# barry-mir/mixing-style-transfer

Measured on AMD Instinct MI355X. Metric: triplets/sec (10 s @ 44.1 kHz, 4-stem, bs=24), higher is better.
Workload: dtype f32

## Files before the change

mixing-style-transfer_amd/csrc/encoder.hip:

```cpp
#include "common.h"

#include <cmath>
#include <type_traits>
#include <vector>

namespace {

typedef float f32x4 __attribute__((ext_vector_type(4)));
constexpr int kConvThreads = 512;
constexpr int kConvWaves = 8;

struct FilmParams {
  const float* feats;
  const float *w0t, *b0, *w3t, *b3, *hwt, *hb;
  const float *s1, *t1, *s2, *t2;
  float* film;
  float2* aff1;
  float2* aff2;
  int Fd, H, nsub;
};

#ifndef MST_FILM_U
#define MST_FILM_U 4
#endif
// ... 90 lines not shown
  static constexpr int RL = 16;
};

template <int SUB>
struct CC<3, SUB> {
  static constexpr int CIN = 64, COUT = 32, NCH = 16, MT = 5, NT = 2;
  static constexpr int WIN = 10, WPG = 2;
  static constexpr int TROWS = 2, TCOLS = 40;
  static constexpr int PR = TROWS + 6, PC = TCOLS + 6;
  static constexpr int RL = 64;
};

template <int SUB>
struct CC<4, SUB> {
  static constexpr int CIN = 32, COUT = 64, NCH = 8, MT = 5, NT = 4;
  static constexpr int WIN = 10, WPG = 2;
  static constexpr int TROWS = 2, TCOLS = 40;
  static constexpr int PR = TROWS + 6, PC = TCOLS + 6;
  static constexpr int RL = 64;
};

struct ConvParams {
  const float* in;
  const float* wfrag;
  const float2* aff;
  float* out;
  int B, nsub;
  int in_rows, in_cols;
  int in_cstride;
  int in_bandoff;
  long long in_clipstride;
  int out_rows, out_cols;
  int tiles_r, tiles_c;
  int sets_per_band;
  float* yraw;
  mst::DetAcc* stats;
  const float* bias;
  int raw_rows, raw_cols;
  const unsigned char* mask;
  float mask_scale;
  int acc_tr, acc_tc, row_off;
  const float* f16_scale;
  const float* f16_winv;
  int pool_h;
  int clip_major;
  _Float16* yraw16;
  const float* y_scale;
  const void* in_lo;
  int cm_mels, cm_overlap;
};

typedef _Float16 h16x4 __attribute__((ext_vector_type(4)));
__device__ __forceinline__ size_t yvec(size_t unit, int t, int nvec) {
  return (unit & ~(size_t)63) * nvec + (size_t)t * 64 + (unit & 63);
}
template <int NV>
__device__ __forceinline__ void load_unit(const void* yraw, const float* y_scale, int band, size_t unit, float (&v)[NV]) {
  if (y_scale) {
    const float inv = y_scale[band * 2 + 1];
    const h16x4* s = reinterpret_cast<const h16x4*>(yraw);
#pragma unroll
    for (int t = 0; t < NV / 4; ++t) {
      const h16x4 q = s[yvec(unit, t, NV / 4)];
#pragma unroll
      for (int r = 0; r < 4; ++r) v[4 * t + r] = (float)q[r] * inv;
    }
// ... 58 lines not shown
  constexpr int WBP = GEO::WBP, PATCH = GEO::PATCH, NWF = GEO::NWF, NPF = GEO::NPF, NCV = GEO::NCV;
  constexpr bool BL = LAYER == 2;
  constexpr int NPFK = BL ? 16 : NPF;
  constexpr int NPIECE = NPFK + NWF, PPT = (NPIECE + 48) / 49;
  extern __shared__ __attribute__((aligned(16))) float smem[];
  const int tid = threadIdx.x, lane = tid & 63;
  const int wave = __builtin_amdgcn_readfirstlane(tid >> 6);
  float* wbuf = smem;
  float* pbuf = smem + 2 * WBP + wave * PATCH;

  const int G = gridDim.x;
  const int wg = mst::xcd_remap(blockIdx.x, G);
  const int total_sets = p.nsub * p.sets_per_band;
  constexpr bool CONTIG = MODE == 1 || MODE == 3;
  const int s_first = CONTIG ? (int)((long long)wg * total_sets / G) : wg;
  const int my_sets = CONTIG ? (int)((long long)(wg + 1) * total_sets / G) - s_first
                             : (wg < total_sets ? (total_sets - wg + G - 1) / G : 0);
  const int nq = my_sets * NCH;
  const int tpb = p.tiles_r * p.tiles_c;

  auto decode = [&](int q) __attribute__((always_inline)) {
    const int s = CONTIG ? min(s_first + q / NCH, total_sets - 1) : wg + (q / NCH) * G;
    Tile t;
    t.band = min(s / p.sets_per_band, p.nsub - 1);
    const int idx = (s - t.band * p.sets_per_band) * kConvWaves + wave;
    t.valid = (q < nq) && idx < p.B * tpb;
    t.clip = t.valid ? idx / tpb : 0;
    const int ti = t.valid ? idx - t.clip * tpb : 0;
    t.tc = ti / p.tiles_r;
    t.tr = ti - t.tc * p.tiles_r;
    return t;
  };

  constexpr bool TS = LAYER == 2 && MODE == 0;
  const int kq = lane >> 4, ai = lane & 15, ag = ai >> 2, areg = ai & 3;
  int abase[MT];
#pragma unroll
  for (int t = 0; t < MT; ++t) {
    int dr, wc;
    if constexpr (GEO1) {
      const int e = 4 * t + areg, wv = e / C::WIN, pos = e % C::WIN;
      dr = pos / 5;
      wc = 5 * (C::WPG * ag + wv) + pos % 5;
    } else {
      dr = TS ? 2 * t + (ag >> 1) : 4 * (ag >> 1) + t;
      wc = 4 * (ag & 1) + areg;
    }
    abase[t] = kq * (PR * PC) + dr * PC + wc;
  }

  f32x4 wreg[NWF];
  float pf[NPFK];
  unsigned long long rowmask = 0;
  unsigned colmask = 0;
  int coff[NCV];
  const float* nsrc = p.in;
  const f32x4* nwsrc = reinterpret_cast<const f32x4*>(p.wfrag);
  int nrow0 = 0, ncol0 = 0, nvalid = 0;
  __amdgpu_buffer_rsrc_t nrsrc = __builtin_amdgcn_make_buffer_rsrc(const_cast<float*>(p.in), 0, 0, 0x00020000);
  __amdgpu_buffer_rsrc_t nwrsrc = __builtin_amdgcn_make_buffer_rsrc(const_cast<float*>(p.wfrag), 0, 0, 0x00020000);
  unsigned nvoff[4] = {0, 0, 0, 0}, nsoff[4] = {0, 0, 0, 0};

  auto prefetch_setup = [&](int q, const Tile& t) __attribute__((always_inline)) {
    const int chunk = q % NCH;
    nwsrc = reinterpret_cast<const f32x4*>(p.wfrag + ((size_t)t.band * NCH + chunk) * WBP);
    nrow0 = (GEO1 ? C::TROWS * t.tr : 8 * t.tr) + (MODE == 3 ? p.row_off : 0) - 3;
    ncol0 = C::TCOLS * t.tc - 3;
    nvalid = t.valid;
    nsrc = p.in + (size_t)t.clip * p.in_clipstride + (size_t)t.band * p.in_bandoff + (size_t)(4 * chunk) * p.in_cstride;
    rowmask = 0, colmask = 0;
    if constexpr (BL) {
      nrsrc = __builtin_amdgcn_make_buffer_rsrc(const_cast<float*>(nsrc), 0, (unsigned)(4 * p.in_cstride) * 4u, 0x00020000);
      nwrsrc = __builtin_amdgcn_make_buffer_rsrc(const_cast<f32x4*>(nwsrc), 0, (unsigned)WBP * 4u, 0x00020000);
      if (chunk == 0) {
        const int rs = lane >> 4, col = lane & 15, cin = ncol0 + col;
        const bool col_in = nvalid && col < PC && cin >= 0 && cin < p.in_cols;
        const int cbase = max(ncol0, 0);
#pragma unroll
// ... 27 lines not shown
        const int row = i / NCV, j = i % NCV;
        const int cc = row / PR, r = row % PR;
        const int rin = nrow0 + r;
        const int rc = min(max(rin, 0), p.in_rows - 1);
        if (nvalid && rin == rc) rowmask |= 1ull << i;
        const float* rowp = nsrc + (size_t)cc * p.in_cstride + (size_t)rc * p.in_cols;
        pf[i] = rowp[coff[j]];
      } else {
        const int e = lane + 64 * i;
        const int row = e / RL, col = e % RL;
        const int cc = min(row / PR, 3), r = row % PR;
        const int rin = nrow0 + r, cin = ncol0 + col;
        const int rc = min(max(rin, 0), p.in_rows - 1), cl = min(max(cin, 0), p.in_cols - 1);
        if (nvalid && row < 4 * PR && col < PC && rin == rc && cin == cl) colmask |= 1u << i;
        pf[i] = nsrc[cc * p.in_cstride + rc * p.in_cols + cl];
      }
    } else if (i < NPIECE) {
      wreg[i - NPF] = nwsrc[tid + kConvThreads * (i - NPF)];
    }
  };

  f32x4 acc[MT][NT];
  double st[NT][2];
  int st_band = -1;
#pragma unroll
  for (int n = 0; n < NT; ++n) st[n][0] = st[n][1] = 0.0;
  Tile cur{}, nxt{};
  nxt = decode(0);
  if (nq > 0) {
    prefetch_setup(0, nxt);
#pragma unroll
    for (int i = 0; i < NPIECE; ++i) prefetch_piece(i);
  }
#ifdef MST_TRACE
  long long trc[5] = {0, 0, 0, 0, 0};
  const long long trc_start = clock64();
#endif
  for (int q = 0; q < nq; ++q) {
    float* wb = wbuf + (q & 1) * WBP;
#ifdef MST_TRACE
    const long long tq0 = clock64();
#endif
#pragma unroll
    for (int i = 0; i < NWF; ++i) reinterpret_cast<f32x4*>(wb)[tid + kConvThreads * i] = wreg[i];
    if constexpr (BL) {
#pragma unroll
      for (int i = 0; i < NPFK; ++i) {
        const int rs = lane >> 4, col = lane & 15, r = 4 * (i & 3) + rs;
        if (r < PR && col < PC) pbuf[((i >> 2) * PR + r) * PC + col] = pf[i];
      }
    } else
#pragma unroll
    for (int i = 0; i < NPF; ++i) {
      if constexpr (RL >= 64) {
        const int row = i / NCV, j = i % NCV, col = lane + 64 * j;
        const bool ok = ((rowmask >> i) & 1ull) && ((colmask >> j) & 1u);
        if (col < PC) pbuf[row * PC + col] = ok ? pf[i] : 0.f;
      } else {
        const int e = lane + 64 * i;
        const int row = e / RL, col = e % RL;
        if (row < 4 * PR && col < PC) pbuf[row * PC + col] = ((colmask >> i) & 1u) ? pf[i] : 0.f;
      }
    }
#ifdef MST_TRACE
    asm volatile("s_waitcnt lgkmcnt(0)" ::: "memory");
    const long long tq1 = clock64();
#endif
    __syncthreads();
#ifdef MST_TRACE
    const long long tq2 = clock64();
    trc[0] += tq1 - tq0, trc[1] += tq2 - tq1, trc[4] += 1;
#endif
    cur = nxt;
    if (!BL || (q + 1) % NCH == 0) nxt = decode(q + 1);
    prefetch_setup(q + 1, nxt);
    const int chunk = q % NCH;
    if (chunk == 0) {
#pragma unroll
      for (int t = 0; t < MT; ++t)
#pragma unroll
        for (int n = 0; n < NT; ++n) acc[t][n] = f32x4{0.f, 0.f, 0.f, 0.f};
    }
    {
      float a[2][MT], b[2][NT];
#pragma unroll
      for (int t = 0; t < MT; ++t) a[0][t] = pbuf[abase[t]];
#pragma unroll
      for (int n = 0; n < NT; ++n) b[0][n] = wb[n * 64 + lane];
      auto taps = [&](auto LO_, auto HI_, auto SKIP_) __attribute__((always_inline)) {
        constexpr int LO = decltype(LO_)::value, HI = decltype(HI_)::value;
        constexpr bool SKIP0 = decltype(SKIP_)::value;
#pragma unroll
        for (int tap = LO; tap < HI; ++tap) {
          const int cu = tap & 1, nx = cu ^ 1;
          const int off = ((tap + 1) / 7) * PC + ((tap + 1) % 7);
#pragma unroll
          for (int i = 0; i < MT * NT; ++i) {
            const int t = i / NT, n = i % NT;
            if (!(SKIP0 && t == 0)) acc[t][n] = __builtin_amdgcn_mfma_f32_16x16x4f32(a[cu][t], b[cu][n], acc[t][n], 0, 0, 0);
            if (tap + 1 < 49) {
              if (i < NT) b[nx][i] = wb[((tap + 1) * NT + i) * 64 + lane];
              else if (i < MT + NT) a[nx][i - NT] = pbuf[abase[i - NT] + off];
            }
            if (i >= MT + NT && i - (MT + NT) < PPT) prefetch_piece(tap * PPT + (i - (MT + NT)));
            __builtin_amdgcn_sched_barrier(0);
          }
        }
      };
      using I0 = std::integral_constant<int, 0>;
      using I14 = std::integral_constant<int, 14>;
      using I49 = std::integral_constant<int, 49>;
      if constexpr (TS) {
        if (cur.tr == 0) taps(I0{}, I14{}, std::true_type{});
        else taps(I0{}, I14{}, std::false_type{});
        taps(I14{}, I49{}, std::false_type{});
      } else {
        taps(I0{}, I49{}, std::false_type{});
      }
    }
#ifdef MST_TRACE
    trc[2] += clock64() - tq2;
#endif
    if (MODE == 1 && chunk == NCH - 1 && cur.valid) {
      const int j = lane & 15, g = lane >> 4;
      if (cur.band != st_band) {
        if (st_band >= 0) flush_stats<NT, C::COUT>(st, p.stats, st_band, lane);
        st_band = cur.band;
      }
      float* yb = p.yraw + ((((size_t)cur.clip * p.nsub + cur.band) * p.acc_tr + cur.tr) * p.acc_tc + cur.tc) *
                               (size_t)(NT * 64 * 4 * MT);
#pragma unroll
      for (int n = 0; n < NT; ++n) {
        const float b = p.bias[cur.band * C::COUT + n * 16 + j];
        f32x4* dst = reinterpret_cast<f32x4*>(yb) + (size_t)n * (64 * MT) + lane;
#pragma unroll
        for (int t = 0; t < MT; ++t) {
          f32x4 v = acc[t][n];
#pragma unroll
          for (int r = 0; r < 4; ++r) {
            v[r] += b;
            int row, col;
            if constexpr (LAYER == 1) {
              const int e = 4 * t + r, wv = e / C::WIN, pos = e % C::WIN;
              row = C::TROWS * cur.tr + pos / 5, col = C::TCOLS * cur.tc + 5 * (C::WPG * g + wv) + pos % 5;
            } else {
              row = 8 * cur.tr + 4 * (g >> 1) + t, col = 8 * cur.tc + 4 * (g & 1) + r;
            }
            if (row < p.raw_rows && col < p.raw_cols) st[n][0] += (double)v[r], st[n][1] += (double)v[r] * (double)v[r];
          }
          dst[64 * t] = v;
        }
      }
    }
    if (MODE == 3 && chunk == NCH - 1 && cur.valid) {
      const int j = lane & 15, g = lane >> 4;
// ... 32 lines not shown
          const int wv = e / C::WIN, pos = e % C::WIN;
          const int row = C::TROWS * cur.tr + pos / 5, col = C::TCOLS * cur.tc + 5 * (C::WPG * g + wv) + pos % 5;
          if (row < p.raw_rows && col < p.raw_cols) {
            const size_t o = (size_t)row * p.raw_cols + col;
            float v = acc[e >> 2][n][e & 3];
            if (mb) v = mb[o] ? v * p.mask_scale : 0.f;
            ob[o] = v;
          }
        }
      }
    }
    if (MODE == 0 && chunk == NCH - 1 && cur.valid) {
      const int j = lane & 15, g = lane >> 4;
      const float2* aff = p.aff + ((size_t)cur.clip * p.nsub + cur.band) * C::COUT;
#pragma unroll
      for (int n = 0; n < NT; ++n) {
        const int ch = n * 16 + j;
        const float2 ac = aff[ch];
        if constexpr (LAYER == 1) {
#pragma unroll
          for (int wv = 0; wv < C::WPG; ++wv) {
            float m = 0.f;
#pragma unroll
            for (int pos = 0; pos < C::WIN; ++pos) {
              const int e = wv * C::WIN + pos;
              m = fmaxf(m, fmaf(acc[e >> 2][n][e & 3], ac.x, ac.y));
            }
            const int pc = 4 * C::WPG * cur.tc + C::WPG * g + wv;
            if (pc < p.out_cols)
              p.out[((((size_t)cur.clip * p.nsub + cur.band) * C::COUT + ch) * p.out_rows + cur.tr) * p.out_cols + pc] = m;
          }
        } else {
          float m = 0.f;
          if constexpr (TS) {
            float m0 = 0.f, m1 = 0.f;
#pragma unroll
            for (int r = 0; r < 4; ++r) {
              m0 = fmaxf(m0, fmaxf(fmaf(acc[0][n][r], ac.x, ac.y), fmaf(acc[1][n][r], ac.x, ac.y)));
              m1 = fmaxf(m1, fmaxf(fmaf(acc[2][n][r], ac.x, ac.y), fmaf(acc[3][n][r], ac.x, ac.y)));
            }
            m0 = fmaxf(m0, __shfl_xor(m0, 32, 64));
            m1 = fmaxf(m1, __shfl_xor(m1, 32, 64));
            m = (g >> 1) ? m1 : m0;
          } else {
#pragma unroll
            for (int t = 0; t < MT; ++t)
#pragma unroll
              for (int r = 0; r < 4; ++r) m = fmaxf(m, fmaf(acc[t][n][r], ac.x, ac.y));
          }
          const int pr = 2 * cur.tr + (g >> 1), pc = 2 * cur.tc + (g & 1);
          if (pr < p.out_rows && pc < p.out_cols)
            p.out[(((size_t)cur.clip * p.nsub + cur.band) * C::COUT + ch) * p.out_rows * p.out_cols +
                  (size_t)pr * p.out_cols + pc] = m;
        }
      }
    }
  }
#ifdef MST_TRACE
  if (MODE == 0 && LAYER == 2 && lane == 0 && p.yraw) {
    float* o = p.yraw + (blockIdx.x * kConvWaves + wave) * 8;
    for (int i = 0; i < 5; ++i) o[i] = (float)trc[i];
    o[5] = (float)(clock64() - trc_start);
  }
#endif
  if ((MODE == 1 || MODE == 3) && st_band >= 0) flush_stats<NT, C::COUT>(st, p.stats, st_band, lane);
}

template <int SUB, int MODE = 0, int LAY = 0>
__global__ __launch_bounds__(kConvThreads) void conv1_resident_kernel(const ConvParams p) {
  using C = CC<1, SUB>;
  constexpr int MT = C::MT, NT = C::NT, PR = C::PR, PC = C::PC;
  static_assert(C::RL == 64, "resident conv1 expects one loader row per instruction");
  static_assert(LAY == 0 || PR == 8, "the channel-minor loader maps lane bits 1..3 to the 8 patch rows");
  constexpr int WCH = 49 * NT * 64;
  constexpr int WBP = ConvGeom<1, SUB>::WBP;
  constexpr int CHS = PR * PC;
  constexpr int PATCH = 8 * CHS;
  constexpr int NPF = LAY == 0 ? 8 * PR : (PC + 3) / 4;
  extern __shared__ __attribute__((aligned(16))) float smem[];
  const int tid = threadIdx.x, lane = tid & 63;
  const int wave = __builtin_amdgcn_readfirstlane(tid >> 6);
  float* wres = smem;
  float* pbuf = smem + 2 * WCH + wave * PATCH;
  constexpr bool DYN = MODE == 0;
  constexpr int kTickets = 16;
  __shared__ unsigned tickets[kTickets];
#ifdef MST_TRACE
  long long trc[5] = {0, 0, 0, 0, 0};
  const long long trc_start = clock64();
#endif

  const int G = gridDim.x;
  const int wg = mst::xcd_remap(blockIdx.x, G);
  const int total_sets = (p.clip_major ? (p.B + p.clip_major - 1) / p.clip_major : 1) * p.nsub * p.sets_per_band;
  const int s_begin = (int)((long long)wg * total_sets / G), s_end = (int)((long long)(wg + 1) * total_sets / G);
  const int tpb = p.tiles_r * p.tiles_c;

  auto decode = [&](int s) __attribute__((always_inline)) {
    Tile t;
    int ti;
    if (p.clip_major) {
      const int ngrp = (p.B + p.clip_major - 1) / p.clip_major;
      const int gb = min(s / p.sets_per_band, ngrp * p.nsub - 1);
      const int idx = (s - gb * p.sets_per_band) * kConvWaves + wave;
      const int grp = gb / p.nsub, c0 = grp * p.clip_major;
      t.band = gb - grp * p.nsub;
      t.valid = (s < s_end) && idx < min(p.clip_major, p.B - c0) * tpb;
      const int cl = t.valid ? idx / tpb : 0;
      t.clip = c0 + cl;
      ti = t.valid ? idx - cl * tpb : 0;
    } else {
      t.band = min(s / p.sets_per_band, p.nsub - 1);
      const int idx = (s - t.band * p.sets_per_band) * kConvWaves + wave;
      t.valid = (s < s_end) && idx < p.B * tpb;
      t.clip = t.valid ? idx / tpb : 0;
      ti = t.valid ? idx - t.clip * tpb : 0;
    }
    t.tc = ti / p.tiles_r;
    t.tr = ti - t.tc * p.tiles_r;
    return t;
  };

  const int kq = lane >> 4, ai = lane & 15, ag = ai >> 2, areg = ai & 3;
  int abase[MT];
#pragma unroll
  for (int t = 0; t < MT; ++t) {
    const int e = 4 * t + areg, wv = e / C::WIN, pos = e % C::WIN;
    abase[t] = kq * CHS + (pos / 5) * PC + 5 * (C::WPG * ag + wv) + pos % 5;
  }

  typename std::conditional<LAY == 0, float, f32x4>::type pf[NPF];
  unsigned long long rowmask = 0;
  bool col_ok = false;
  int coff = 0, nrow0 = 0, nvalid = 0;
  const float* nsrc = p.in;
  bool nfast = false;
  __amdgpu_buffer_rsrc_t nrsrc = __builtin_amdgcn_make_buffer_rsrc(const_cast<float*>(p.in), 0, 0, 0x00020000);
  unsigned nsoff = 0, nvoff = 0;
  static_assert(WBP - WCH >= 4, "the chunk pitch leaves at least 16 zero bytes behind the weights");
  const float* const zero16 = p.wfrag + WCH;
  const int lr = (lane >> 1) & 7, lhalf = lane & 1, lfq = lane >> 4;
  const unsigned frame_bytes = (unsigned)p.cm_mels * 32u;
  auto prefetch_setup = [&](const Tile& t) __attribute__((always_inline)) {
    nrow0 = C::TROWS * t.tr - 3;
    nvalid = t.valid;
    rowmask = 0;
    if constexpr (LAY == 0) {
      const int col0 = C::TCOLS * t.tc - 3, cin = col0 + lane;
      nsrc = p.in + (size_t)t.clip * p.in_clipstride + (size_t)t.band * p.in_bandoff;
      col_ok = lane < PC && cin >= 0 && cin < p.in_cols;
      coff = min(max(cin, 0), p.in_cols - 1);
    } else {
      const int rin = nrow0 + lr, rc = min(max(rin, 0), p.in_rows - 1);
      nsrc = p.in + (size_t)t.clip * p.in_clipstride;
      col_ok = nvalid && rin == rc;
      coff = ((t.band * p.cm_overlap + rc) * 8 + 4 * lhalf) * 4;
      nrow0 = C::TCOLS * t.tc - 3 + lfq;
      if constexpr (DYN) {
        const int f0 = C::TCOLS * t.tc - 3;
        nfast = nvalid && f0 >= 0 && f0 + 4 * NPF + 3 < p.in_cols;
        nrsrc = __builtin_amdgcn_make_buffer_rsrc(const_cast<float*>(nsrc), 0, (unsigned)p.in_cols * frame_bytes, 0x00020000);
// ... 199 lines not shown
            }
          } else {
            float m = 0.f;
#pragma unroll
            for (int pos = 0; pos < C::WIN; ++pos) {
              const int e = wv * C::WIN + pos;
              m = fmaxf(m, fmaf(acc[e >> 2][n][e & 3], ac.x, ac.y));
            }
            if (pc < p.out_cols) orow[(size_t)ch * p.out_rows * p.out_cols + pc] = m;
          }
        }
      }
    }
#ifdef MST_TRACE
    trc[1] += clock64() - tr1;
#endif
  };
  f32x4 sav[MT][NT];
  float2 sav_ac[NT];
  Tile prev{};
#pragma unroll
  for (int t = 0; t < MT; ++t)
#pragma unroll
    for (int n = 0; n < NT; ++n) sav[t][n] = f32x4{0.f, 0.f, 0.f, 0.f};
#pragma unroll
  for (int n = 0; n < NT; ++n) sav_ac[n] = float2{0.f, 0.f};
  auto epi_part = [&](auto N_, auto WV_) __attribute__((always_inline)) {
    constexpr int n = decltype(N_)::value, wv = decltype(WV_)::value;
    const int j = lane & 15, g = lane >> 4;
    const int ch = n * 16 + j;
    float* orow = p.out + ((size_t)prev.clip * p.nsub + prev.band) * C::COUT * p.out_rows * p.out_cols + (size_t)prev.tr * p.out_cols;
    const float2 ac = sav_ac[n];
    const int pc = 4 * C::WPG * prev.tc + C::WPG * g + wv;
    if (SUB == 2 && p.pool_h == 1) {
#pragma unroll
      for (int hr = 0; hr < 2; ++hr) {
        float m = 0.f;
#pragma unroll
        for (int pos = 0; pos < 5; ++pos) {
          const int e = wv * C::WIN + 5 * hr + pos;
          m = fmaxf(m, fmaf(sav[e >> 2][n][e & 3], ac.x, ac.y));
        }
        if (prev.valid && pc < p.out_cols && 2 * prev.tr + hr < p.out_rows)
          orow[(size_t)ch * p.out_rows * p.out_cols + (size_t)(prev.tr + hr) * p.out_cols + pc] = m;
      }
    } else {
      float m = 0.f;
#pragma unroll
      for (int pos = 0; pos < C::WIN; ++pos) {
        const int e = wv * C::WIN + pos;
        m = fmaxf(m, fmaf(sav[e >> 2][n][e & 3], ac.x, ac.y));
      }
      if (prev.valid && pc < p.out_cols) orow[(size_t)ch * p.out_rows * p.out_cols + pc] = m;
    }
  };
  auto tile_dyn = [&]() __attribute__((always_inline)) {
#ifdef MST_TRACE
    const long long tr0 = clock64();
#endif
    float2 e_ac[NT];
    {
      const float2* aff = p.aff + ((size_t)cur.clip * p.nsub + cur.band) * C::COUT;
#pragma unroll
      for (int n = 0; n < NT; ++n) e_ac[n] = aff[n * 16 + (lane & 15)];
    }
    {
      constexpr int kEpi0 = 12;
      const bool skip_c = cur.tr == 0, skip_b = 2 * cur.tr + 2 >= p.in_rows;
      const int next_off = skip_b ? 0 : 5 * PC, next_w = skip_b ? 0 : 35 * NT * 64;
      float a[2][MT], b[2][NT];
#pragma unroll
      for (int t = 0; t < MT; ++t) a[0][t] = pbuf[abase[t] + 2 * PC];
#pragma unroll
      for (int n = 0; n < NT; ++n) b[0][n] = wres[(14 * NT + n) * 64 + lane];
      auto kstep = [&](auto S_) __attribute__((always_inline)) {
        constexpr int ks = decltype(S_)::value;
        constexpr int cu = ks & 1, nx = cu ^ 1;
        constexpr bool last = ks == 41 || ks == 69 || ks == 97;
        constexpr int s1 = ks + 1, l1 = s1 < 42 ? s1 : s1 < 70 ? s1 - 42 : s1 - 70;
        constexpr int row1 = (s1 < 42 ? 2 : s1 < 70 ? 5 : 0) + l1 / 14, tap1 = 7 * row1 + (l1 % 14) / 2, ch1 = l1 & 1;
        constexpr int off1 = ch1 * 4 * CHS + row1 * PC + (l1 % 14) / 2;
#pragma unroll
        for (int i = 0; i < MT * NT; ++i) {
          const int t = i / NT, n = i % NT;
          acc[t][n] = __builtin_amdgcn_mfma_f32_16x16x4f32(a[cu][t], b[cu][n], ks == 0 ? f32x4{0.f, 0.f, 0.f, 0.f} : acc[t][n], 0, 0, 0);
          if constexpr (!last) {
            if (i < NT) b[nx][i] = wres[ch1 * WCH + (tap1 * NT + i) * 64 + lane];
            else if (i < MT + NT) a[nx][i - NT] = pbuf[abase[i - NT] + off1];
          } else if constexpr (ks == 41) {
            if (i < NT) b[nx][i] = wres[next_w + i * 64 + lane];
            else if (i < MT + NT) a[nx][i - NT] = pbuf[abase[i - NT] + next_off];
          } else if constexpr (ks == 69) {
            if (i < NT) b[nx][i] = wres[i * 64 + lane];
            else if (i < MT + NT) a[nx][i - NT] = pbuf[abase[i - NT]];
          }
          if (i == MT + NT) {
            if constexpr (LAY == 0) {
              if constexpr (ks >= 8 && ks < 8 + NPF / 2) prefetch_piece(2 * (ks - 8)), prefetch_piece(2 * (ks - 8) + 1);
            } else {
              if constexpr (ks >= 8 && ks % 2 == 0 && ks / 2 - 4 < NPF) prefetch_piece(ks / 2 - 4);
            }
          }
          if (i == MT + NT + 1) {
            if constexpr (ks == 0) ticket_issue();
            if constexpr (ks == 6) {
              nxt = ticket_take();
              nxt_seg = dseg;
              prefetch_setup(nxt);
            }
            if constexpr (ks >= kEpi0 && ks < kEpi0 + 2 * NT * C::WPG && (ks - kEpi0) % 2 == 0)
              epi_part(std::integral_constant<int, (ks - kEpi0) / 2 / C::WPG>{}, std::integral_constant<int, (ks - kEpi0) / 2 % C::WPG>{});
          }
          __builtin_amdgcn_sched_barrier(0);
        }
      };
      static_assert(LAY == 0 ? 8 + NPF / 2 <= 42 : 2 * (NPF + 3) < 42, "the patch fetch must fit block A");
      static_for<42>([&](auto I) __attribute__((always_inline)) { kstep(std::integral_constant<int, decltype(I)::value>{}); });
      if (!skip_b) static_for<28>([&](auto I) __attribute__((always_inline)) { kstep(std::integral_constant<int, 42 + decltype(I)::value>{}); });
      if (!skip_c) static_for<28>([&](auto I) __attribute__((always_inline)) { kstep(std::integral_constant<int, 70 + decltype(I)::value>{}); });
    }
    {
      const float bz = wres[lane];
#pragma unroll
      for (int t = 0; t < MT; ++t)
#pragma unroll
        for (int n = 0; n < NT; ++n) sav[t][n] = __builtin_amdgcn_mfma_f32_16x16x4f32(0.f, bz, acc[t][n], 0, 0, 0);
    }
#pragma unroll
    for (int n = 0; n < NT; ++n) sav_ac[n] = e_ac[n];
    prev = cur;
#ifdef MST_TRACE
    trc[0] += clock64() - tr0, trc[4] += 1;
#endif
  };
  auto load_band = [&](int band) __attribute__((always_inline)) {
    for (int c = 0; c < 2; ++c) {
      const f32x4* src = reinterpret_cast<const f32x4*>(p.wfrag + ((size_t)band * 2 + c) * WBP);
      for (int k = tid; k < WCH / 4; k += kConvThreads) reinterpret_cast<f32x4*>(wres + c * WCH)[k] = src[k];
    }
  };
  if constexpr (DYN) {
    for (int k = 0; k < nseg; ++k) {
#ifdef MST_TRACE
      const long long tb0 = clock64();
#endif
      __syncthreads();
      load_band((gb0 + k) % p.nsub);
      if (tid == 0) tickets[(k + kTickets - 1) % kTickets] = 0;
      __syncthreads();
#ifdef MST_TRACE
      trc[3] += clock64() - tb0;
#endif
// ... 2415 lines not shown
        static int calls = 0;
        if (++calls == 10) {
          (void)hipDeviceSynchronize();
          std::vector<float> h(256 * kConvWaves * 8);
          (void)hipMemcpy(h.data(), trace_buf, h.size() * sizeof(float), hipMemcpyDeviceToHost);
          for (int w = 0; w < kConvWaves; ++w) {
            double a[6] = {0, 0, 0, 0, 0, 0};
            for (int b = 0; b < g; ++b)
              for (int i = 0; i < 6; ++i) a[i] += h[(b * kConvWaves + w) * 8 + i] / g;
            fprintf(stderr, "trace wave %d: tiles %.1f  k-steps %.0f (%.0f per tile)  wait for the patch loads %.0f (%.0f)  stage %.0f (%.0f)  barriers %.0f  total %.0f\n",
                    w, a[4], a[0], a[0] / a[4], a[1], a[1] / a[4], a[2], a[2] / a[4], a[3], a[5]);
          }
        }
      }
#endif
      err = hipGetLastError();
    } else {
      err = e->sub == 2 ? launch_conv<1, 2>(cp, g, st) : launch_conv<1, 1>(cp, g, st);
    }
    if (err != hipSuccess) return mst::fail(MST_EHIP, "conv1 launch failed: %s", hipGetErrorString(err));
  }
  mark(2);
  {
    ConvParams cp{};
    cp.in = pool1, cp.wfrag = e->w2frag, cp.aff = aff2, cp.out = pool_in, cp.B = B, cp.nsub = ns;
    cp.in_rows = e->H1, cp.in_cols = L.W1;
    cp.in_cstride = e->H1 * L.W1;
    cp.in_bandoff = 32 * e->H1 * L.W1;
    cp.in_clipstride = (long long)ns * 32 * e->H1 * L.W1;
    cp.out_rows = e->FD, cp.out_cols = L.W2;
    cp.tiles_r = (e->FD + 1) / 2;
    cp.tiles_c = (L.W2 + 1) / 2;
    cp.sets_per_band = (B * cp.tiles_r * cp.tiles_c + kConvWaves - 1) / kConvWaves;
    const int g = std::min(grid, ns * cp.sets_per_band);
    hipError_t err;
    if (e->conv1_f16x3 >= 2) {
      constexpr size_t lds = (size_t)(kF16Steps * 4 * 2 * 64 + kConvWaves * 2 * 14 * 14) * 16;
      static unsigned long long attr = 0;
      if (mst::first_use_on_device(attr)) {
        err = hipFuncSetAttribute(reinterpret_cast<const void*>(conv2_f16x3_kernel<3>),
                                  hipFuncAttributeMaxDynamicSharedMemorySize, (int)lds);
        if (err == hipSuccess)
          err = hipFuncSetAttribute(reinterpret_cast<const void*>(conv2_f16x3_kernel<1>),
                                    hipFuncAttributeMaxDynamicSharedMemorySize, (int)lds);
        if (err != hipSuccess) return mst::fail(MST_EHIP, "conv2 f16x3 attribute failed: %s", hipGetErrorString(err));
      }
      cp.f16_scale = reinterpret_cast<const float*>(ws + L.f16scale);
      cp.f16_winv = e->f16_winv2;
      const h16x8* ih = reinterpret_cast<const h16x8*>(ws + L.pool1_h16);
      const h16x8* il = reinterpret_cast<const h16x8*>(ws + L.pool1_l16);
      const h16x8* wf = reinterpret_cast<const h16x8*>(e->w2frag16);
      if (e->conv1_f16x3 == 3) hipLaunchKernelGGL((conv2_f16x3_kernel<1>), dim3(g), dim3(kConvThreads), lds, st, cp, ih, il, wf);
      else hipLaunchKernelGGL((conv2_f16x3_kernel<3>), dim3(g), dim3(kConvThreads), lds, st, cp, ih, il, wf);
      err = hipGetLastError();
    } else {
#ifdef MST_TRACE
      static float* trace_buf2 = nullptr;
      if (!trace_buf2) (void)hipMalloc(&trace_buf2, 256 * kConvWaves * 8 * sizeof(float));
      cp.yraw = trace_buf2;
#endif
      err = launch_conv<2, 2>(cp, g, st);
#ifdef MST_TRACE
      {
        static int calls = 0;
        if (++calls == 10) {
          (void)hipDeviceSynchronize();
          std::vector<float> h(256 * kConvWaves * 8);
          (void)hipMemcpy(h.data(), trace_buf2, h.size() * sizeof(float), hipMemcpyDeviceToHost);
          for (int w = 0; w < kConvWaves; ++w) {
            double a[6] = {0, 0, 0, 0, 0, 0};
            for (int b = 0; b < g; ++b)
              for (int i = 0; i < 6; ++i) a[i] += h[(b * kConvWaves + w) * 8 + i] / g;
            fprintf(stderr, "conv2 trace wave %d: chunks %.1f  staging %.0f (%.0f per chunk)  barrier wait %.0f (%.0f)  taps %.0f (%.0f)  total %.0f\n",
                    w, a[4], a[0], a[0] / a[4], a[1], a[1] / a[4], a[2], a[2] / a[4], a[5]);
          }
        }
      }
#endif
    }
    if (err != hipSuccess) return mst::fail(MST_EHIP, "conv2 launch failed: %s", hipGetErrorString(err));
  }
  mark(3);
  {
    AttnParams ap{pool_in, e->att0frag, e->att0_b, e->att2_w, e->att2_b, scores, B, e->C, L.W2, e->cfg.attn_hidden};
    const int mtiles = (B * L.W2 + 16 * kAttnMT - 1) / (16 * kAttnMT);
    hipLaunchKernelGGL(attn_scores_kernel, dim3(mtiles), dim3(256), 0, st, ap);
    MST_HIP_CHECK(hipGetLastError());
  }
  mark(4);
  {
    float* pooled = reinterpret_cast<float*>(ws + L.pooled);
    PoolParams pp{pool_in, scores, pooled, e->C, L.W2};
    const int slices = (e->C + 127) / 128;
    hipLaunchKernelGGL(attn_pool_kernel, dim3(B, slices), dim3(256), (size_t)((L.W2 + 3) & ~3) * sizeof(float), st, pp);
    MST_HIP_CHECK(hipGetLastError());
    ProjParams pj{pooled, e->projfrag, e->proj_b, emb, B, e->C, e->cfg.embed_dim};
    const int mt_all = (B + 15) / 16;
    if (mt_all <= 1) launch_proj<1>(pj, 1, st);
    else if (mt_all <= 2) launch_proj<2>(pj, 1, st);
    else if (mt_all <= 3) launch_proj<3>(pj, 1, st);
    else if (mt_all <= 5) launch_proj<5>(pj, 1, st);
    else launch_proj<8>(pj, (B + 127) / 128, st);
    MST_HIP_CHECK(hipGetLastError());
  }
  mark(5);
  return MST_OK;
}

namespace {
struct TrainLayout {
  WsLayout base;
// ... 825 lines not shown
```

Baseline: 2779.

## Add row-tiled conv2 eval kernel with per-row boundary MFMA skipping

Replaces the generic conv2 eval path with a dedicated kernel that tiles outputs as 4 rows by 16 columns (plus an edge-column tile variant), and uses a per-tile skip mask to omit MFMAs for taps that read padding rows. The conv1 kernel's tap loop is also split into per-row groups so M-tiles hitting out-of-range rows are skipped, with a row-pure A mapping. Old tap-skip and trace code in the generic kernel are removed. This adds code complexity and new tiling/edge handling that could introduce correctness or scheduling regressions.

Result: no change. 2795, median of 6 (+0.5%).

```diff
diff --git a/mixing-style-transfer_amd/csrc/encoder.hip b/mixing-style-transfer_amd/csrc/encoder.hip
--- a/mixing-style-transfer_amd/csrc/encoder.hip
+++ b/mixing-style-transfer_amd/csrc/encoder.hip
@@ -146,6 +146,7 @@
   long long in_clipstride;
   int out_rows, out_cols;
   int tiles_r, tiles_c;
+  int c2_edge;
   int sets_per_band;
   float* yraw;
   mst::DetAcc* stats;
@@ -270,7 +271,6 @@
     return t;
   };
 
-  constexpr bool TS = LAYER == 2 && MODE == 0;
   const int kq = lane >> 4, ai = lane & 15, ag = ai >> 2, areg = ai & 3;
   int abase[MT];
 #pragma unroll
@@ -281,7 +281,7 @@
       dr = pos / 5;
       wc = 5 * (C::WPG * ag + wv) + pos % 5;
     } else {
-      dr = TS ? 2 * t + (ag >> 1) : 4 * (ag >> 1) + t;
+      dr = 4 * (ag >> 1) + t;
       wc = 4 * (ag & 1) + areg;
     }
     abase[t] = kq * (PR * PC) + dr * PC + wc;
@@ -375,15 +375,8 @@
 #pragma unroll
     for (int i = 0; i < NPIECE; ++i) prefetch_piece(i);
   }
-#ifdef MST_TRACE
-  long long trc[5] = {0, 0, 0, 0, 0};
-  const long long trc_start = clock64();
-#endif
   for (int q = 0; q < nq; ++q) {
     float* wb = wbuf + (q & 1) * WBP;
-#ifdef MST_TRACE
-    const long long tq0 = clock64();
-#endif
 #pragma unroll
     for (int i = 0; i < NWF; ++i) reinterpret_cast<f32x4*>(wb)[tid + kConvThreads * i] = wreg[i];
     if constexpr (BL) {
@@ -405,15 +398,7 @@
         if (row < 4 * PR && col < PC) pbuf[row * PC + col] = ((colmask >> i) & 1u) ? pf[i] : 0.f;
       }
     }
-#ifdef MST_TRACE
-    asm volatile("s_waitcnt lgkmcnt(0)" ::: "memory");
-    const long long tq1 = clock64();
-#endif
     __syncthreads();
-#ifdef MST_TRACE
-    const long long tq2 = clock64();
-    trc[0] += tq1 - tq0, trc[1] += tq2 - tq1, trc[4] += 1;
-#endif
     cur = nxt;
     if (!BL || (q + 1) % NCH == 0) nxt = decode(q + 1);
     prefetch_setup(q + 1, nxt);
@@ -430,17 +415,15 @@
       for (int t = 0; t < MT; ++t) a[0][t] = pbuf[abase[t]];
 #pragma unroll
       for (int n = 0; n < NT; ++n) b[0][n] = wb[n * 64 + lane];
-      auto taps = [&](auto LO_, auto HI_, auto SKIP_) __attribute__((always_inline)) {
-        constexpr int LO = decltype(LO_)::value, HI = decltype(HI_)::value;
-        constexpr bool SKIP0 = decltype(SKIP_)::value;
-#pragma unroll
-        for (int tap = LO; tap < HI; ++tap) {
+      {
+#pragma unroll
+        for (int tap = 0; tap < 49; ++tap) {
           const int cu = tap & 1, nx = cu ^ 1;
           const int off = ((tap + 1) / 7) * PC + ((tap + 1) % 7);
 #pragma unroll
           for (int i = 0; i < MT * NT; ++i) {
             const int t = i / NT, n = i % NT;
-            if (!(SKIP0 && t == 0)) acc[t][n] = __builtin_amdgcn_mfma_f32_16x16x4f32(a[cu][t], b[cu][n], acc[t][n], 0, 0, 0);
+            acc[t][n] = __builtin_amdgcn_mfma_f32_16x16x4f32(a[cu][t], b[cu][n], acc[t][n], 0, 0, 0);
             if (tap + 1 < 49) {
               if (i < NT) b[nx][i] = wb[((tap + 1) * NT + i) * 64 + lane];
               else if (i < MT + NT) a[nx][i - NT] = pbuf[abase[i - NT] + off];
@@ -449,21 +432,8 @@
             __builtin_amdgcn_sched_barrier(0);
           }
         }
-      };
-      using I0 = std::integral_constant<int, 0>;
-      using I14 = std::integral_constant<int, 14>;
-      using I49 = std::integral_constant<int, 49>;
-      if constexpr (TS) {
-        if (cur.tr == 0) taps(I0{}, I14{}, std::true_type{});
-        else taps(I0{}, I14{}, std::false_type{});
-        taps(I14{}, I49{}, std::false_type{});
-      } else {
-        taps(I0{}, I49{}, std::false_type{});
-      }
-    }
-#ifdef MST_TRACE
-    trc[2] += clock64() - tq2;
-#endif
+      }
+    }
     if (MODE == 1 && chunk == NCH - 1 && cur.valid) {
       const int j = lane & 15, g = lane >> 4;
       if (cur.band != st_band) {
@@ -562,22 +532,10 @@
           }
         } else {
           float m = 0.f;
-          if constexpr (TS) {
-            float m0 = 0.f, m1 = 0.f;
-#pragma unroll
-            for (int r = 0; r < 4; ++r) {
-              m0 = fmaxf(m0, fmaxf(fmaf(acc[0][n][r], ac.x, ac.y), fmaf(acc[1][n][r], ac.x, ac.y)));
-              m1 = fmaxf(m1, fmaxf(fmaf(acc[2][n][r], ac.x, ac.y), fmaf(acc[3][n][r], ac.x, ac.y)));
-            }
-            m0 = fmaxf(m0, __shfl_xor(m0, 32, 64));
-            m1 = fmaxf(m1, __shfl_xor(m1, 32, 64));
-            m = (g >> 1) ? m1 : m0;
-          } else {
-#pragma unroll
-            for (int t = 0; t < MT; ++t)
-#pragma unroll
-              for (int r = 0; r < 4; ++r) m = fmaxf(m, fmaf(acc[t][n][r], ac.x, ac.y));
-          }
+#pragma unroll
+          for (int t = 0; t < MT; ++t)
+#pragma unroll
+            for (int r = 0; r < 4; ++r) m = fmaxf(m, fmaf(acc[t][n][r], ac.x, ac.y));
           const int pr = 2 * cur.tr + (g >> 1), pc = 2 * cur.tc + (g & 1);
           if (pr < p.out_rows && pc < p.out_cols)
             p.out[(((size_t)cur.clip * p.nsub + cur.band) * C::COUT + ch) * p.out_rows * p.out_cols +
@@ -586,14 +544,202 @@
       }
     }
   }
-#ifdef MST_TRACE
-  if (MODE == 0 && LAYER == 2 && lane == 0 && p.yraw) {
-    float* o = p.yraw + (blockIdx.x * kConvWaves + wave) * 8;
-    for (int i = 0; i < 5; ++i) o[i] = (float)trc[i];
-    o[5] = (float)(clock64() - trc_start);
-  }
-#endif
   if ((MODE == 1 || MODE == 3) && st_band >= 0) flush_stats<NT, C::COUT>(st, p.stats, st_band, lane);
+}
+
+struct Conv2Rows {
+  static constexpr int MT = 4, NT = 4, NCH = 8;
+  static constexpr int PC = 24, PR = 14, CHS = PR * PC, PATCH = 4 * CHS;
+  static constexpr int NB = 5;
+  static constexpr int WBP = ConvGeom<2, 2>::WBP, NWF = ConvGeom<2, 2>::NWF;
+  static constexpr size_t LDS = (size_t)(2 * WBP + kConvWaves * PATCH) * sizeof(float);
+  static constexpr bool can_skip(int dr, int t) { return t + dr < 3 || t + dr >= 7; }
+  static_assert(CHS % 64 == 16, "k-groups on disjoint banks");
+  static_assert(LDS <= 160 * 1024, "conv2 eval: LDS");
+};
+
+__global__ __launch_bounds__(kConvThreads) void conv2_rows_kernel(const ConvParams p) {
+  using K = Conv2Rows;
+  constexpr int MT = K::MT, NT = K::NT, NCH = K::NCH, PC = K::PC, CHS = K::CHS, NB = K::NB, WBP = K::WBP, NWF = K::NWF;
+  constexpr int NPFK = 4 * NB, NPIECE = NPFK + NWF;
+  static_assert(NPIECE <= 49, "one prefetch piece per tap");
+  extern __shared__ __attribute__((aligned(16))) float smem[];
+  const int tid = threadIdx.x, lane = tid & 63;
+  const int wave = __builtin_amdgcn_readfirstlane(tid >> 6);
+  float* wbuf = smem;
+  float* pbuf = smem + 2 * WBP + wave * K::PATCH;
+
+  const int G = gridDim.x;
+  const int wg = mst::xcd_remap(blockIdx.x, G);
+  const int total_sets = p.nsub * p.sets_per_band;
+  const int my_sets = wg < total_sets ? (total_sets - wg + G - 1) / G : 0;
+  const int nq = my_sets * NCH;
+  const int nfull = p.tiles_r * p.tiles_c, tpb = nfull + (p.c2_edge ? (p.tiles_r + 1) >> 1 : 0);
+  const int slot = wave < 4 ? wave : wave ^ 1;
+
+  auto decode = [&](int q) __attribute__((always_inline)) {
+    const int s = wg + (q / NCH) * G;
+    Tile t;
+    t.band = min(s / p.sets_per_band, p.nsub - 1);
+    const int idx = (s - t.band * p.sets_per_band) * kConvWaves + slot;
+    t.valid = (q < nq) && idx < p.B * tpb;
+    t.clip = t.valid ? idx / tpb : 0;
+    const int ti = t.valid ? idx - t.clip * tpb : 0;
+    if (ti < nfull) {
+      t.tc = ti / p.tiles_r;
+      t.tr = ti - t.tc * p.tiles_r;
+    } else {
+      t.tc = p.tiles_c;
+      t.tr = 2 * (ti - nfull);
+    }
+    return t;
+  };
+
+  const int kq = lane >> 4, ai = lane & 15;
+  int abase[MT];
+
+  f32x4 wreg[NWF];
+  float pf[NPFK];
+  __amdgpu_buffer_rsrc_t nrsrc = __builtin_amdgcn_make_buffer_rsrc(const_cast<float*>(p.in), 0, 0, 0x00020000);
+  __amdgpu_buffer_rsrc_t nwrsrc = __builtin_amdgcn_make_buffer_rsrc(const_cast<float*>(p.wfrag), 0, 0, 0x00020000);
+  unsigned nvoff[NB], nsoff[NB];
+  int nlds[NB];
+#pragma unroll
+  for (int b = 0; b < NB; ++b) nvoff[b] = 0x80000000u, nsoff[b] = 0, nlds[b] = -1;
+
+  auto prefetch_setup = [&](int q, const Tile& t) __attribute__((always_inline)) {
+    const int chunk = q % NCH;
+    const float* src = p.in + (size_t)t.clip * p.in_clipstride + (size_t)t.band * p.in_bandoff + (size_t)(4 * chunk) * p.in_cstride;
+    const float* wsrc = p.wfrag + ((size_t)t.band * NCH + chunk) * WBP;
+    nrsrc = __builtin_amdgcn_make_buffer_rsrc(const_cast<float*>(src), 0, (unsigned)(4 * p.in_cstride) * 4u, 0x00020000);
+    nwrsrc = __builtin_amdgcn_make_buffer_rsrc(const_cast<float*>(wsrc), 0, (unsigned)WBP * 4u, 0x00020000);
+    if (chunk == 0) {
+      const bool edge = t.tc == p.tiles_c;
+      const int row0 = 4 * t.tr - 3, col0 = 16 * t.tc - 3;
+      const int lrow = edge ? lane >> 4 : lane >> 5, lcol = edge ? lane & 15 : lane & 31;
+      const int rpb = edge ? 4 : 2, nrows = edge ? 14 : 10, ncols = edge ? 14 : 22;
+      const int cin = col0 + lcol;
+      const bool col_in = t.valid && lcol < ncols && cin >= 0 && cin < p.in_cols;
+      const int cbase = max(col0, 0);
+#pragma unroll
+      for (int b = 0; b < NB; ++b) {
+        const int r = rpb * b + lrow, rin = row0 + r, rbase = min(max(row0 + rpb * b, 0), p.in_rows - 1);
+        const bool ok = col_in && r < nrows && rin >= 0 && rin < p.in_rows;
+        nsoff[b] = (unsigned)(rbase * p.in_cols + cbase) * 4u;
+        nvoff[b] = ok ? (unsigned)((rin - rbase) * p.in_cols + (cin - cbase)) * 4u : 0x80000000u;
+        nlds[b] = (r < nrows && lcol < ncols) ? r * PC + lcol : -1;
+      }
+    }
+  };
+  auto prefetch_piece = [&](int i) __attribute__((always_inline)) {
+    if (i < NPFK) {
+      pf[i] = __builtin_bit_cast(float, __builtin_amdgcn_raw_buffer_load_b32(nrsrc, nvoff[i % NB], nsoff[i % NB] + (unsigned)((i / NB) * p.in_cstride) * 4u, 0));
+    } else if (i < NPIECE) {
+      wreg[i - NPFK] = __builtin_bit_cast(f32x4, __builtin_amdgcn_raw_buffer_load_b128(nwrsrc, (unsigned)tid * 16u, (unsigned)(kConvThreads * (i - NPFK)) * 16u, 0));
+    }
+  };
+
+  f32x4 acc[MT][NT];
+  Tile cur{}, nxt{};
+  nxt = decode(0);
+  if (nq > 0) {
+    prefetch_setup(0, nxt);
+#pragma unroll
+    for (int i = 0; i < NPIECE; ++i) prefetch_piece(i);
+  }
+  bool cur_edge = false;
+  unsigned skipmask = 0;
+  for (int q = 0; q < nq; ++q) {
+    float* wb = wbuf + (q & 1) * WBP;
+#pragma unroll
+    for (int i = 0; i < NWF; ++i) reinterpret_cast<f32x4*>(wb)[tid + kConvThreads * i] = wreg[i];
+#pragma unroll
+    for (int b = 0; b < NB; ++b)
+      if (nlds[b] >= 0) {
+#pragma unroll
+        for (int c = 0; c < 4; ++c) pbuf[c * CHS + nlds[b]] = pf[c * NB + b];
+      }
+    __syncthreads();
+    cur = nxt;
+    if ((q + 1) % NCH == 0) nxt = decode(q + 1);
+    prefetch_setup(q + 1, nxt);
+    const int chunk = q % NCH;
+    if (chunk == 0) {
+      cur_edge = cur.tc == p.tiles_c;
+#pragma unroll
+      for (int t = 0; t < MT; ++t) {
+        abase[t] = kq * CHS + (cur_edge ? (t + 4 * (ai >> 3)) * PC + (ai & 7) : t * PC + ai);
+#pragma unroll
+        for (int n = 0; n < NT; ++n) acc[t][n] = f32x4{0.f, 0.f, 0.f, 0.f};
+      }
+      skipmask = 0;
+#pragma unroll
+      for (int dr = 0; dr < 7; ++dr)
+#pragma unroll
+        for (int t = 0; t < MT; ++t) {
+          const int rin = 4 * cur.tr + t + dr - 3;
+          if (Conv2Rows::can_skip(dr, t) && !cur_edge && (rin < 0 || rin >= p.in_rows)) skipmask |= 1u << (4 * dr + t);
+        }
+    }
+    {
+      float a[2][MT], b[2][NT];
+#pragma unroll
+      for (int t = 0; t < MT; ++t) a[0][t] = pbuf[abase[t]];
+#pragma unroll
+      for (int n = 0; n < NT; ++n) b[0][n] = wb[n * 64 + lane];
+      auto side = [&](int tap, int i) __attribute__((always_inline)) {
+        const int nx = (tap & 1) ^ 1, off = ((tap + 1) / 7) * PC + ((tap + 1) % 7);
+        if (tap + 1 < 49) {
+          if (i < NT) b[nx][i] = wb[((tap + 1) * NT + i) * 64 + lane];
+          else if (i < MT + NT) a[nx][i - NT] = pbuf[abase[i - NT] + off];
+        }
+        if (i == MT + NT) prefetch_piece(tap);
+      };
+      static_for<7>([&](auto D) __attribute__((always_inline)) {
+        constexpr int DR = decltype(D)::value;
+#pragma unroll
+        for (int tap = 7 * DR; tap < 7 * DR + 7; ++tap) {
+          const int cu = tap & 1;
+#pragma unroll
+          for (int t = 0; t < MT; ++t) {
+            if (Conv2Rows::can_skip(DR, t)) {
+              if (!((skipmask >> (4 * DR + t)) & 1u)) {
+#pragma unroll
+                for (int n = 0; n < NT; ++n) acc[t][n] = __builtin_amdgcn_mfma_f32_16x16x4f32(a[cu][t], b[cu][n], acc[t][n], 0, 0, 0);
+              }
+#pragma unroll
+              for (int n = 0; n < NT; ++n) side(tap, t * NT + n);
+              __builtin_amdgcn_sched_barrier(0);
+            } else {
+#pragma unroll
+              for (int n = 0; n < NT; ++n) {
+                acc[t][n] = __builtin_amdgcn_mfma_f32_16x16x4f32(a[cu][t], b[cu][n], acc[t][n], 0, 0, 0);
+                side(tap, t * NT + n);
+                __builtin_amdgcn_sched_barrier(0);
+              }
+            }
+          }
+        }
+      });
+    }
+    if (chunk == NCH - 1 && cur.valid) {
+      const int j = lane & 15, g = lane >> 4;
+      const float2* aff = p.aff + ((size_t)cur.clip * p.nsub + cur.band) * 64;
+      const int pr = cur_edge ? cur.tr + (g >> 1) : cur.tr, pc = cur_edge ? 4 * p.tiles_c + (g & 1) : 4 * cur.tc + g;
+#pragma unroll
+      for (int n = 0; n < NT; ++n) {
+        const int ch = n * 16 + j;
+        const float2 ac = aff[ch];
+        float m = 0.f;
+#pragma unroll
+        for (int t = 0; t < MT; ++t)
+#pragma unroll
+          for (int r = 0; r < 4; ++r) m = fmaxf(m, fmaf(acc[t][n][r], ac.x, ac.y));
+        if (pr < p.out_rows && pc < p.out_cols)
+          p.out[(((size_t)cur.clip * p.nsub + cur.band) * 64 + ch) * p.out_rows * p.out_cols + (size_t)pr * p.out_cols + pc] = m;
+      }
+    }
+  }
 }
 
 template <int SUB, int MODE = 0, int LAY = 0>
@@ -651,12 +797,19 @@
     return t;
   };
 
+  constexpr bool ROWMAP = DYN;
+  static_assert(!ROWMAP || SUB == 2, "the row-pure M-tiles are those of the 2 x 40 tile");
   const int kq = lane >> 4, ai = lane & 15, ag = ai >> 2, areg = ai & 3;
   int abase[MT];
 #pragma unroll
   for (int t = 0; t < MT; ++t) {
-    const int e = 4 * t + areg, wv = e / C::WIN, pos = e % C::WIN;
-    abase[t] = kq * CHS + (pos / 5) * PC + 5 * (C::WPG * ag + wv) + pos % 5;
+    if constexpr (ROWMAP) {
+      const int row = t < 4 ? t >> 1 : areg >> 1, wv = t < 4 ? t & 1 : areg & 1, pos = t < 4 ? areg : 4;
+      abase[t] = kq * CHS + row * PC + 5 * (C::WPG * ag + wv) + pos;
+    } else {
+      const int e = 4 * t + areg, wv = e / C::WIN, pos = e % C::WIN;
+      abase[t] = kq * CHS + (pos / 5) * PC + 5 * (C::WPG * ag + wv) + pos % 5;
+    }
   }
 
   typename std::conditional<LAY == 0, float, f32x4>::type pf[NPF];
@@ -922,25 +1075,20 @@
     float* orow = p.out + ((size_t)prev.clip * p.nsub + prev.band) * C::COUT * p.out_rows * p.out_cols + (size_t)prev.tr * p.out_cols;
     const float2 ac = sav_ac[n];
     const int pc = 4 * C::WPG * prev.tc + C::WPG * g + wv;
+    auto row_max = [&](int hr, float m) __attribute__((always_inline)) {
+#pragma unroll
+      for (int r = 0; r < 4; ++r) m = fmaxf(m, fmaf(sav[2 * hr + wv][n][r], ac.x, ac.y));
+      return fmaxf(m, fmaf(sav[4][n][2 * hr + wv], ac.x, ac.y));
+    };
     if (SUB == 2 && p.pool_h == 1) {
 #pragma unroll
       for (int hr = 0; hr < 2; ++hr) {
-        float m = 0.f;
-#pragma unroll
-        for (int pos = 0; pos < 5; ++pos) {
-          const int e = wv * C::WIN + 5 * hr + pos;
-          m = fmaxf(m, fmaf(sav[e >> 2][n][e & 3], ac.x, ac.y));
-        }
+        const float m = row_max(hr, 0.f);
         if (prev.valid && pc < p.out_cols && 2 * prev.tr + hr < p.out_rows)
           orow[(size_t)ch * p.out_rows * p.out_cols + (size_t)(prev.tr + hr) * p.out_cols + pc] = m;
       }
     } else {
-      float m = 0.f;
-#pragma unroll
-      for (int pos = 0; pos < C::WIN; ++pos) {
-        const int e = wv * C::WIN + pos;
-        m = fmaxf(m, fmaf(sav[e >> 2][n][e & 3], ac.x, ac.y));
-      }
+      const float m = row_max(1, row_max(0, 0.f));
       if (prev.valid && pc < p.out_cols) orow[(size_t)ch * p.out_rows * p.out_cols + pc] = m;
     }
   };
@@ -957,14 +1105,17 @@
     {
       constexpr int kEpi0 = 12;
       const bool skip_c = cur.tr == 0, skip_b = 2 * cur.tr + 2 >= p.in_rows;
+      const bool skip_lo2 = skip_c, skip_lo0 = 2 * cur.tr < 3, skip_hi4 = skip_b, skip_hi6 = 2 * cur.tr + 4 >= p.in_rows;
       const int next_off = skip_b ? 0 : 5 * PC, next_w = skip_b ? 0 : 35 * NT * 64;
       float a[2][MT], b[2][NT];
 #pragma unroll
       for (int t = 0; t < MT; ++t) a[0][t] = pbuf[abase[t] + 2 * PC];
 #pragma unroll
       for (int n = 0; n < NT; ++n) b[0][n] = wres[(14 * NT + n) * 64 + lane];
-      auto kstep = [&](auto S_) __attribute__((always_inline)) {
+      auto kstep = [&](auto S_, auto V_) __attribute__((always_inline)) {
         constexpr int ks = decltype(S_)::value;
+        constexpr int V = decltype(V_)::value;
+        constexpr int NA = V == 0 ? MT : MT - 2;
         constexpr int cu = ks & 1, nx = cu ^ 1;
         constexpr bool last = ks == 41 || ks == 69 || ks == 97;
         constexpr int s1 = ks + 1, l1 = s1 < 42 ? s1 : s1 < 70 ? s1 - 42 : s1 - 70;
@@ -972,8 +1123,13 @@
         constexpr int off1 = ch1 * 4 * CHS + row1 * PC + (l1 % 14) / 2;
 #pragma unroll
         for (int i = 0; i < MT * NT; ++i) {
-          const int t = i / NT, n = i % NT;
-          acc[t][n] = __builtin_amdgcn_mfma_f32_16x16x4f32(a[cu][t], b[cu][n], ks == 0 ? f32x4{0.f, 0.f, 0.f, 0.f} : acc[t][n], 0, 0, 0);
+          if (i < NA * NT) {
+            const int ta = i / NT, t = V == 1 ? ta + 2 : V == 2 && ta == 2 ? 4 : ta, n = i % NT;
+            acc[t][n] = __builtin_amdgcn_mfma_f32_16x16x4f32(a[cu][t], b[cu][n], ks == 0 ? f32x4{0.f, 0.f, 0.f, 0.f} : acc[t][n], 0, 0, 0);
+          }
+          if constexpr (ks == 0 && V == 1) {
+            if (i >= NA * NT) acc[(i - NA * NT) / NT][(i - NA * NT) % NT] = f32x4{0.f, 0.f, 0.f, 0.f};
+          }
           if constexpr (!last) {
             if (i < NT) b[nx][i] = wres[ch1 * WCH + (tap1 * NT + i) * 64 + lane];
             else if (i < MT + NT) a[nx][i - NT] = pbuf[abase[i - NT] + off1];
@@ -1005,9 +1161,29 @@
         }
       };
       static_assert(LAY == 0 ? 8 + NPF / 2 <= 42 : 2 * (NPF + 3) < 42, "the patch fetch must fit block A");
-      static_for<42>([&](auto I) __attribute__((always_inline)) { kstep(std::integral_constant<int, decltype(I)::value>{}); });
-      if (!skip_b) static_for<28>([&](auto I) __attribute__((always_inline)) { kstep(std::integral_constant<int, 42 + decltype(I)::value>{}); });
-      if (!skip_c) static_for<28>([&](auto I) __attribute__((always_inline)) { kstep(std::integral_constant<int, 70 + decltype(I)::value>{}); });
+      auto tap_row = [&](auto LO_, auto V_) __attribute__((always_inline)) {
+        static_for<14>([&](auto I) __attribute__((always_inline)) {
+          kstep(std::integral_constant<int, decltype(LO_)::value + decltype(I)::value>{}, V_);
+        });
+      };
+      using V0 = std::integral_constant<int, 0>;
+      using V1 = std::integral_constant<int, 1>;
+      using V2 = std::integral_constant<int, 2>;
+#define MST_TAP_ROW(LO, COND, V) \
+  if (COND) tap_row(std::integral_constant<int, LO>{}, V{}); \
+  else tap_row(std::integral_constant<int, LO>{}, V0{})
+      MST_TAP_ROW(0, skip_lo2, V1);
+      tap_row(std::integral_constant<int, 14>{}, V0{});
+      MST_TAP_ROW(28, skip_hi4, V2);
+      if (!skip_b) {
+        tap_row(std::integral_constant<int, 42>{}, V0{});
+        MST_TAP_ROW(56, skip_hi6, V2);
+      }
+      if (!skip_c) {
+        MST_TAP_ROW(70, skip_lo0, V1);
+        tap_row(std::integral_constant<int, 84>{}, V0{});
+      }
+#undef MST_TAP_ROW
     }
     {
       const float bz = wres[lane];
@@ -3489,6 +3665,13 @@
     cp.tiles_r = (e->FD + 1) / 2;
     cp.tiles_c = (L.W2 + 1) / 2;
     cp.sets_per_band = (B * cp.tiles_r * cp.tiles_c + kConvWaves - 1) / kConvWaves;
+    if (e->conv1_f16x3 < 2) {
+      cp.tiles_r = e->FD;
+      cp.tiles_c = L.W2 / 4 + (L.W2 % 4 == 3 ? 1 : 0);
+      cp.c2_edge = L.W2 % 4 == 1 || L.W2 % 4 == 2;
+      const int tpb = cp.tiles_r * cp.tiles_c + (cp.c2_edge ? (cp.tiles_r + 1) / 2 : 0);
+      cp.sets_per_band = (B * tpb + kConvWaves - 1) / kConvWaves;
+    }
     const int g = std::min(grid, ns * cp.sets_per_band);
     hipError_t err;
     if (e->conv1_f16x3 >= 2) {
@@ -3511,29 +3694,14 @@
       else hipLaunchKernelGGL((conv2_f16x3_kernel<3>), dim3(g), dim3(kConvThreads), lds, st, cp, ih, il, wf);
       err = hipGetLastError();
     } else {
-#ifdef MST_TRACE
-      static float* trace_buf2 = nullptr;
-      if (!trace_buf2) (void)hipMalloc(&trace_buf2, 256 * kConvWaves * 8 * sizeof(float));
-      cp.yraw = trace_buf2;
-#endif
-      err = launch_conv<2, 2>(cp, g, st);
-#ifdef MST_TRACE
-      {
-        static int calls = 0;
-        if (++calls == 10) {
-          (void)hipDeviceSynchronize();
-          std::vector<float> h(256 * kConvWaves * 8);
-          (void)hipMemcpy(h.data(), trace_buf2, h.size() * sizeof(float), hipMemcpyDeviceToHost);
-          for (int w = 0; w < kConvWaves; ++w) {
-            double a[6] = {0, 0, 0, 0, 0, 0};
-            for (int b = 0; b < g; ++b)
-              for (int i = 0; i < 6; ++i) a[i] += h[(b * kConvWaves + w) * 8 + i] / g;
-            fprintf(stderr, "conv2 trace wave %d: chunks %.1f  staging %.0f (%.0f per chunk)  barrier wait %.0f (%.0f)  taps %.0f (%.0f)  total %.0f\n",
-                    w, a[4], a[0], a[0] / a[4], a[1], a[1] / a[4], a[2], a[2] / a[4], a[5]);
-          }
-        }
-      }
-#endif
+      static unsigned long long attr = 0;
+      if (mst::first_use_on_device(attr)) {
+        err = hipFuncSetAttribute(reinterpret_cast<const void*>(conv2_rows_kernel), hipFuncAttributeMaxDynamicSharedMemorySize,
+                                  (int)Conv2Rows::LDS);
+        if (err != hipSuccess) return mst::fail(MST_EHIP, "conv2 attribute failed: %s", hipGetErrorString(err));
+      }
+      hipLaunchKernelGGL(conv2_rows_kernel, dim3(g), dim3(kConvThreads), Conv2Rows::LDS, st, cp);
+      err = hipGetLastError();
     }
     if (err != hipSuccess) return mst::fail(MST_EHIP, "conv2 launch failed: %s", hipGetErrorString(err));
   }
```
